# 2025-comprehensive-design/AudioLDM-with-LoRA

Hardware: AMD Instinct MI355X
Metric: unet_denoise_steps_per_sec (higher is better)
Workload: dtype bf16; 1 GPU; audioldm-s-full-v2 UNet + rank-4 LoRA (q,k,v,out), DDIM 200-step schedule, batch 4 x 10 s clips (latent 250x16), CFG 2.5 (UNet batch 8), bf16; per_gpu_batch=4, parallelism=prompt-sharded x1, hip_graph=True, graph_chains=1

## Files before the change

### audioldm_with_lora_amd/csrc/attention.hip

```cpp
#include "common.h"
#include <cstdlib>
#include <type_traits>

#ifndef ATTN_ML
#define ATTN_ML 0
#endif
#ifndef ATTN_FENCE
#define ATTN_FENCE 0
#endif

namespace {

constexpr int KV = 64;
constexpr int VS = 136;
constexpr int VS8 = 72;


typedef float f32x2 __attribute__((ext_vector_type(2)));
constexpr float RESCALE_THR = 5.0f;

__device__ __forceinline__ float max3f(float a, float b, float c) {
  float d;
  asm("v_max3_f32 %0, %1, %2, %3" : "=v"(d) : "v"(a), "v"(b), "v"(c));
  return d;
}

template <int DP, bool FP8 = false>
struct AttnCfg {
  static constexpr int DK = DP / 16;
  static constexpr bool VL = DP % 32 == 0;
  static constexpr int DT = VL ? DP / 32 : DP / 32 + 1;
  static constexpr int ONES_T = VL ? 0 : DP / 32;
  static constexpr int ONES_I = 4 * ((DP % 32) >> 3);
  static_assert(DP % 16 == 0, "row DP must land on hh = 0, register 4 * (row / 8)");
  static constexpr int KS = FP8 ? DP + 8 : DP * 2 + (((DP / 8) % 2 == 0) ? 16 : 0);
  static constexpr int VSB = FP8 ? VS8 : VS;
  static constexpr int KBYTES = KV * KS;
  static constexpr int VBYTES = DT * 32 * VSB;
  static constexpr int TILE = KBYTES + VBYTES;
};

template <int DP, int NW, int SP, bool PRESCALED, bool FP8 = false, bool LSE = false>
__global__ __launch_bounds__(64 * NW) void attention_kernel(const bf16* __restrict__ q, int ldq,
                                                            const bf16* __restrict__ k, int ldk,
                                                            const bf16* __restrict__ vt, int vt_ld, long long vt_bs,
                                                            int N, int D, float c ,
                                                            bf16* __restrict__ out, int out_ld, float* __restrict__ lse,
                                                            const int* __restrict__ kv_len) {
  aldm_touch_kernargs<96>();
#ifndef ALDM_NO_KA_PREFETCH
  aldm_prefetch_next_kernargs<96>(threadIdx.x);
#endif
  using Cfg = AttnCfg<DP, FP8>;
  constexpr int T = 64 * NW;
  constexpr int DK = Cfg::DK, DT = Cfg::DT, KS = Cfg::KS, VS = Cfg::VSB;
#ifndef ATTN_FP8_PBIAS
#define ATTN_FP8_PBIAS 8.f
#endif
  constexpr float PBIAS = FP8 ? ATTN_FP8_PBIAS : 0.f;
  using frag_t = std::conditional_t<FP8, long, bf16x8>;
  constexpr int KCH = KV * (DP / 8);
  constexpr int VCH = DP * (KV / 8);
  constexpr int KPT = (KCH + T - 1) / T, VPT = (VCH + T - 1) / T;
  constexpr int QW = NW / SP;
  static_assert(NW % SP == 0, "waves must divide into key groups");

  extern __shared__ __attribute__((aligned(16))) char smem[];
  char* Ks = smem;
  char* Vs = smem + 2 * SP * Cfg::KBYTES;

  const int tid = threadIdx.x, lane = tid & 63, wave = tid >> 6;
  const int r = lane & 31, hh = lane >> 5;
  int qblk = blockIdx.x, head = blockIdx.y, b = blockIdx.z;
  {
    const int nq = gridDim.x, H = gridDim.y, npairs = H * gridDim.z;
    if ((npairs & 7) == 0) {
      const int L = blockIdx.x + nq * (blockIdx.y + H * blockIdx.z);
      const int xcd = L & 7, slot = L >> 3;
      const int pl = slot / nq;
      qblk = slot - pl * nq;
      const int pair = pl * 8 + xcd;
      b = pair / H;
      head = pair - b * H;
    }
  }
  const int grp = wave / QW;
  const int q0 = (qblk * QW + (wave - grp * QW)) * 32;
  const bf16* qb = q + (long long)b * N * ldq + head * D;
  const bf16* kb = k + (long long)b * N * ldk + head * D;
  const bf16* vb = vt + (long long)b * vt_bs + (long long)head * D * vt_ld;
  const bf16x8 zero8 = {0, 0, 0, 0, 0, 0, 0, 0};
  const int Nk = kv_len ? max(1, min(kv_len[b], N)) : N;
  if (kv_len && qblk * QW * 32 >= Nk) {
    for (int i = tid; i < QW * 32 * (D / 4); i += T) {
      const int row = qblk * QW * 32 + i / (D / 4), c4 = i % (D / 4);
      if (row < N) *reinterpret_cast<uint2*>(out + ((long long)b * N + row) * out_ld + head * D + c4 * 4) = make_uint2(0u, 0u);
    }
    return;
  }

  {
    const int npad = DT * 32 - D;
    for (int i = tid; i < 2 * SP * npad * (VS / 8); i += T) {
      const int buf = i / (npad * (VS / 8)), rem = i - buf * npad * (VS / 8);
      const unsigned fill = (!Cfg::VL && D + rem / (VS / 8) == DP) ? (FP8 ? 0x38383838u : 0x3F803F80u) : 0u;
      reinterpret_cast<uint2*>(Vs + buf * Cfg::VBYTES + D * VS)[rem] = make_uint2(fill, fill);
    }
  }

  frag_t qf[DK];
#pragma unroll
  for (int ks = 0; ks < DK; ++ks) {
    const int col = 16 * ks + 8 * hh;
    const bf16x8 qv = (q0 + r < N && col < D) ? *reinterpret_cast<const bf16x8*>(qb + (long long)(q0 + r) * ldq + col) : zero8;
    if constexpr (FP8) { const uint2 f = bf16x8_to_fp8(qv); qf[ks] = pack2(f.x, f.y); }
    else qf[ks] = qv;
  }

  bf16x8 kreg[2][SP][KPT], vreg[2][SP][VPT];
  constexpr unsigned OOB = 0x80000000u;
  unsigned k_off[KPT], v_off[VPT];
#pragma unroll
  for (int i = 0; i < KPT; ++i) {
    const int cidx = tid + i * T;
    const int row = cidx / (DP / 8), ch = cidx - row * (DP / 8);
    k_off[i] = (cidx < KCH && ch * 8 < D) ? (unsigned)row * (unsigned)(ldk * 2) + ch * 16 : OOB;
  }
#pragma unroll
  for (int i = 0; i < VPT; ++i) {
    const int cidx = tid + i * T;
    const int row = cidx >> 3, ch = cidx & 7;
    v_off[i] = (cidx < VCH && row < D) ? (unsigned)row * (unsigned)(vt_ld * 2) + ch * 16 : OOB;
  }
  auto prefetch_k = [&](int kvbase, auto setc) {
   constexpr int SET = decltype(setc)::value;
#pragma unroll
   for (int j = 0; j < SP; ++j) {
    const int kv0 = kvbase + j * KV;
    const int bytes = max(0, ((Nk - kv0 - 1) * ldk + D) * 2);
    const __amdgpu_buffer_rsrc_t rs = __builtin_amdgcn_make_buffer_rsrc(const_cast<bf16*>(kb + (long long)kv0 * ldk), 0, kv0 < Nk ? bytes : 0, 0x00020000);
#pragma unroll
    for (int i = 0; i < KPT; ++i) kreg[SET][j][i] = __builtin_bit_cast(bf16x8, __builtin_amdgcn_raw_buffer_load_b128(rs, k_off[i], 0, 0));
   }
  };
  auto prefetch_v = [&](int kvbase, auto setc) {
   constexpr int SET = decltype(setc)::value;
#pragma unroll
   for (int j = 0; j < SP; ++j) {
    const int kv0 = kvbase + j * KV;
    const int bytes = max(0, (D * vt_ld - kv0) * 2);
    const __amdgpu_buffer_rsrc_t rs = __builtin_amdgcn_make_buffer_rsrc(const_cast<bf16*>(vb + kv0), 0, kv0 < Nk ? bytes : 0, 0x00020000);
#pragma unroll
    for (int i = 0; i < VPT; ++i) vreg[SET][j][i] = __builtin_bit_cast(bf16x8, __builtin_amdgcn_raw_buffer_load_b128(rs, v_off[i], 0, 0));
   }
  };
  auto prefetch = [&](int kvbase, auto setc) { prefetch_k(kvbase, setc); prefetch_v(kvbase, setc); };
  auto stage_k = [&](int buf, auto setc) {
   constexpr int SET = decltype(setc)::value;
#pragma unroll
   for (int j = 0; j < SP; ++j) {
#pragma unroll
    for (int i = 0; i < KPT; ++i) {
      const int cidx = tid + i * T;
      const int row = cidx / (DP / 8), ch = cidx - row * (DP / 8);
      if (cidx < KCH) {
        if constexpr (FP8) *reinterpret_cast<uint2*>(Ks + (buf * SP + j) * Cfg::KBYTES + row * KS + ch * 8) = bf16x8_to_fp8(kreg[SET][j][i]);
        else *reinterpret_cast<bf16x8*>(Ks + (buf * SP + j) * Cfg::KBYTES + row * KS + ch * 16) = kreg[SET][j][i];
      }
    }
   }
  };
  auto stage_v = [&](int buf, auto setc, int kvbase) {
   constexpr int SET = decltype(setc)::value;
#pragma unroll
   for (int j = 0; j < SP; ++j) {
    const int kv0 = kvbase + j * KV;
#pragma unroll
    for (int i = 0; i < VPT; ++i) {
      const int cidx = tid + i * T;
      const int row = cidx >> 3, ch = cidx & 7;
      if (cidx < VCH) {
        bf16x8 v = vreg[SET][j][i];
        if (kv0 + KV > Nk) {
#pragma unroll
          for (int e = 0; e < 8; ++e) if (kv0 + ch * 8 + e >= Nk) v[e] = (bf16)0.f;
        }
        if constexpr (FP8) {
          *reinterpret_cast<uint2*>(Vs + (buf * SP + j) * Cfg::VBYTES + row * VS + ch * 8) = bf16x8_to_fp8(v);
        } else {
          uint2* dst = reinterpret_cast<uint2*>(Vs + (buf * SP + j) * Cfg::VBYTES + row * VS + ch * 16);
          const uint4 u = __builtin_bit_cast(uint4, v);
          dst[0] = make_uint2(u.x, u.y);
          dst[1] = make_uint2(u.z, u.w);
        }
      }
    }
   }
  };
  auto stage = [&](int buf, auto setc, int kvbase) { stage_k(buf, setc); stage_v(buf, setc, kvbase); };

  f32x16 o[DT];
#pragma unroll
  for (int t = 0; t < DT; ++t)
#pragma unroll
    for (int i = 0; i < 16; ++i) o[t][i] = 0.f;
  float m_run = 0.f;
  constexpr bool ML = Cfg::VL && ATTN_ML;
  constexpr bool LSUM = LSE && !Cfg::VL;
  static_assert(!(LSE && (FP8 || PRESCALED)), "the lse form is the plain bf16 kernel");
  float l_run = 0.f;
  f32x2 l_pk = {0.f, 0.f};
  f32x16 lacc;
#pragma unroll
  for (int i = 0; i < 16; ++i) lacc[i] = 0.f;
  const bf16x8 ones8 = {(bf16)1.f, (bf16)1.f, (bf16)1.f, (bf16)1.f, (bf16)1.f, (bf16)1.f, (bf16)1.f, (bf16)1.f};
  f32x16 minit;
#pragma unroll
  for (int i = 0; i < 16; ++i) minit[i] = 0.f;

  const int ntiles = (Nk + KV - 1) / KV;
  const int niter = (ntiles + SP - 1) / SP;
  using Set0 = std::integral_constant<int, 0>;
  using Set1 = std::integral_constant<int, 1>;

  auto scores = [&](int it, f32x16 (&s)[2]) {
    const int buf = (it & 1) * SP + grp;
#pragma unroll
    for (int sub = 0; sub < 2; ++sub) {
#pragma unroll
      for (int ks = 0; ks < DK; ++ks) {
        if constexpr (FP8) {
          const uint2 kf = *reinterpret_cast<const uint2*>(Ks + buf * Cfg::KBYTES + (sub * 32 + r) * KS + 16 * ks + 8 * hh);
// ... 70 lines not shown
        const uint2 hi = *reinterpret_cast<const uint2*>(vrow + 16);
        return __builtin_bit_cast(bf16x8, make_uint4(lo.x, lo.y, hi.x, hi.y));
      }
    };
    frag_t vf[2][DT];
#pragma unroll
    for (int t = 0; t < DT; ++t) vf[0][t] = vfrag(t, 0);
#pragma unroll
    for (int s2 = 0; s2 < 4; ++s2) {
      const int sub = s2 >> 1, i0 = (s2 & 1) * 8;
      if (s2 + 1 < 4) {
#pragma unroll
        for (int t = 0; t < DT; ++t) vf[(s2 + 1) & 1][t] = vfrag(t, s2 + 1);
      }
      int pw8[2] = {0, 0};
#pragma unroll
      for (int i = 0; i < 8; i += 2) {
        const float e0 = PRESCALED ? s[sub][i0 + i] : fmaf(s[sub][i0 + i], c, PBIAS - m_run);
        const float e1 = PRESCALED ? s[sub][i0 + i + 1] : fmaf(s[sub][i0 + i + 1], c, PBIAS - m_run);
#ifdef ATTN_DIAG_NOEXP
        const float p0 = e0, p1 = e1;
#else
        const float p0 = __builtin_amdgcn_exp2f(e0), p1 = __builtin_amdgcn_exp2f(e1);
#endif
#ifdef ATTN_FP8_CLAMP
        const float p0c = fminf(p0, 448.f), p1c = fminf(p1, 448.f);
#define P0 p0c
#define P1 p1c
#else
#define P0 p0
#define P1 p1
#endif
        if constexpr ((Cfg::VL && !ML) || LSUM) l_pk += f32x2{p0, p1};
        if constexpr (FP8) {
          pw8[i >> 2] = (i & 2) ? __builtin_amdgcn_cvt_pk_fp8_f32(P0, P1, pw8[i >> 2], true) : __builtin_amdgcn_cvt_pk_fp8_f32(P0, P1, pw8[i >> 2], false);
        } else {
          pf[s2][i] = (bf16)p0;
          pf[s2][i + 1] = (bf16)p1;
        }
      }
      if constexpr (FP8) pf[s2] = pack2((unsigned)pw8[0], (unsigned)pw8[1]);
      if (ATTN_FENCE) __builtin_amdgcn_sched_barrier(0);
#pragma unroll
      for (int t = 0; t < DT; ++t) {
        if constexpr (FP8) o[t] = __builtin_amdgcn_mfma_f32_32x32x16_fp8_fp8(vf[s2 & 1][t], pf[s2], o[t], 0, 0, 0);
        else o[t] = __builtin_amdgcn_mfma_f32_32x32x16_bf16(vf[s2 & 1][t], pf[s2], o[t], 0, 0, 0);
      }
      if constexpr (ML && !FP8) lacc = __builtin_amdgcn_mfma_f32_32x32x16_bf16(ones8, pf[s2], lacc, 0, 0, 0);
      if (ATTN_FENCE) __builtin_amdgcn_sched_barrier(0);
    }
  };
  auto mine = [&](int it) { return SP == 1 || (it * SP + grp) * KV < Nk; };

  prefetch(0, Set0{});
  prefetch(SP * KV, Set1{});
  stage(0, Set0{}, 0);
  __builtin_amdgcn_s_waitcnt(0x0F70);
  __syncthreads();
  auto iteration = [&](int it, auto curc) {
    constexpr int CUR = decltype(curc)::value;
    f32x16 s[2];
    const bool me = mine(it);
#if ATTN_FENCE
    if (me) scores(it, s);
    __builtin_amdgcn_sched_barrier(0);
    if (it + 1 < niter) stage((it & 1) ^ 1, std::integral_constant<int, CUR ^ 1>{}, (it + 1) * SP * KV);
    prefetch((it + 2) * SP * KV, curc);
    __builtin_amdgcn_sched_barrier(0);
    if (me) softmax_pv(it, s);
#else
#ifndef ATTN_DIAG_NOLOAD
    prefetch((it + 2) * SP * KV, curc);
#endif
    if (me) {
      scores(it, s);
      softmax_pv(it, s);
    }
#ifndef ATTN_DIAG_NOLOAD
    if (it + 1 < niter) stage((it & 1) ^ 1, std::integral_constant<int, CUR ^ 1>{}, (it + 1) * SP * KV);
#endif
#endif
    __syncthreads();
  };
  for (int it = 0; it < niter; it += 2) {
    iteration(it, Set0{});
    if (it + 1 < niter) iteration(it + 1, Set1{});
  }
  if constexpr ((Cfg::VL && !ML) || LSUM) l_run = l_pk[0] + l_pk[1];

  if constexpr (SP > 1) {
    constexpr int WVALS = DT * 16 + 2;
    float* xch = reinterpret_cast<float*>(smem);
    const bool idle = grp * KV >= Nk;
    if (grp > 0) {
      float* mine = xch + ((grp - 1) * QW + (wave - grp * QW)) * WVALS * 64;
      mine[lane] = idle ? -INFINITY : m_run;
#pragma unroll
      for (int t = 0; t < DT; ++t)
#pragma unroll
        for (int i = 0; i < 16; ++i) mine[(1 + t * 16 + i) * 64 + lane] = o[t][i];
      mine[(1 + DT * 16) * 64 + lane] = ML ? lacc[0] : l_run;
    }
    __syncthreads();
    if (grp > 0) return;
#pragma unroll
    for (int g = 1; g < SP; ++g) {
      const float* peer = xch + ((g - 1) * QW + wave) * WVALS * 64;
      const float m1 = peer[lane];
      const float m_new = fmaxf(m_run, m1);
      const float a0 = __builtin_amdgcn_exp2f(m_run - m_new), a1 = __builtin_amdgcn_exp2f(m1 - m_new);
      m_run = m_new;
#pragma unroll
      for (int t = 0; t < DT; ++t)
#pragma unroll
        for (int i = 0; i < 16; ++i) o[t][i] = o[t][i] * a0 + peer[(1 + t * 16 + i) * 64 + lane] * a1;
      lacc[0] = lacc[0] * a0 + peer[(1 + DT * 16) * 64 + lane] * a1;
      l_run = l_run * a0 + peer[(1 + DT * 16) * 64 + lane] * a1;
    }
  }

  const float l_half = (Cfg::VL && !ML) ? l_run : o[Cfg::ONES_T][Cfg::ONES_I];
  const float l_tot = ML ? lacc[0] : l_half + __shfl_xor(l_half, 32, 64);
  const float inv = 1.0f / l_tot;
  const float l_lse = LSUM ? l_run + __shfl_xor(l_run, 32, 64) : l_tot;
  if (lse && hh == 0 && q0 + r < N)
    lse[((long long)b * gridDim.y + head) * N + q0 + r] = m_run + __log2f(l_lse);
  if (q0 + r < N) {
    bf16* orow = out + ((long long)b * N + q0 + r) * out_ld + head * D;
#pragma unroll
    for (int t = 0; t < (DP + 31) / 32; ++t)
#pragma unroll
      for (int g = 0; g < 4; ++g) {
        const int d0 = t * 32 + 8 * g + 4 * hh;
        if (d0 < D) {
          bf16x4 v = {(bf16)(o[t][4 * g] * inv), (bf16)(o[t][4 * g + 1] * inv), (bf16)(o[t][4 * g + 2] * inv), (bf16)(o[t][4 * g + 3] * inv)};
          *reinterpret_cast<bf16x4*>(orow + d0) = v;
        }
      }
  }
}

template <int DP, int NW, int SP, bool PS, bool FP8 = false, bool LSE = false>
int launch_attn(const void* q, int ldq, const void* k, int ldk, const void* vt, int vt_ld, long long vt_bs, int B, int N,
                int H, int D, float scale, void* out, int out_ld, float* lse, const int* kv_len, hipStream_t st) {
  using Cfg = AttnCfg<DP, FP8>;
  auto kern = attention_kernel<DP, NW, SP, PS, FP8, LSE>;
  constexpr int MERGE = SP == 1 ? 0 : (SP - 1) * (NW / SP) * (Cfg::DT * 16 + 2) * 256;
  constexpr int LDS = 2 * SP * Cfg::TILE > MERGE ? 2 * SP * Cfg::TILE : MERGE;
  static unsigned long long attr_done = 0;
  if (LDS > 48 * 1024)
    if (int rc = aldm_set_max_lds(reinterpret_cast<const void*>(kern), LDS, &attr_done, "attention")) return rc;
  dim3 grid(cdiv(N, 32 * (NW / SP)), H, B);
  hipLaunchKernelGGL(kern, grid, dim3(64 * NW), LDS, st, (const bf16*)q, ldq, (const bf16*)k, ldk, (const bf16*)vt,
                     vt_ld, vt_bs, N, D, scale * 1.44269504088896340736f, (bf16*)out, out_ld, lse, kv_len);
  return aldm_launch_status("attention");
}

template <int DP, bool PS, bool FP8 = false>
int launch_attn_d(const void* q, int ldq, const void* k, int ldk, const void* vt, int vt_ld, long long vt_bs, int B, int N,
                  int H, int D, float scale, void* out, int out_ld, float* lse, const int* kv_len, hipStream_t st) {
#define ALDM_ATTN_ARGS q, ldq, k, ldk, vt, vt_ld, vt_bs, B, N, H, D, scale, out, out_ld, lse, kv_len, st
  if constexpr (FP8) {
    if (N >= 768) {
      if ((long long)cdiv(N, 256) * H * B >= 256) return launch_attn<DP, 8, 1, PS, true>(ALDM_ATTN_ARGS);
      return launch_attn<DP, 8, 2, PS, true>(ALDM_ATTN_ARGS);
    }
    if (N >= 192) return launch_attn<DP, 4, 2, PS, true>(ALDM_ATTN_ARGS);
    if (N >= 64) return launch_attn<DP, 4, 1, PS, true>(ALDM_ATTN_ARGS);
    return launch_attn<DP, 1, 1, PS, true>(ALDM_ATTN_ARGS);
  }
#define ALDM_ATTN_GO(NWV, SPV)                                                              \
  do {                                                                                      \
    if constexpr (!PS && DP % 32 != 0) {                                                    \
      if (lse) return launch_attn<DP, NWV, SPV, PS, false, true>(ALDM_ATTN_ARGS);           \
    }                                                                                       \
    return launch_attn<DP, NWV, SPV, PS>(ALDM_ATTN_ARGS);                                   \
  } while (0)
  static const int force = getenv("ALDM_ATTN_CFG") ? atoi(getenv("ALDM_ATTN_CFG")) : 0;
  if (force == 81) ALDM_ATTN_GO(8, 1);
  if (force == 82) ALDM_ATTN_GO(8, 2);
  if (force == 41) ALDM_ATTN_GO(4, 1);
  if (force == 42) ALDM_ATTN_GO(4, 2);
  if (force == 21) ALDM_ATTN_GO(2, 1);
  if constexpr (DP == 32) {
    if (force == 162) return launch_attn<DP, 16, 2, PS>(ALDM_ATTN_ARGS);
  }
  if (N >= 768) {
    if ((long long)cdiv(N, 256) * H * B >= 256) ALDM_ATTN_GO(8, 1);
    ALDM_ATTN_GO(8, 2);
  }
  if (N >= 192) ALDM_ATTN_GO(4, 2);
  if (N >= 64) ALDM_ATTN_GO(4, 1);
  ALDM_ATTN_GO(1, 1);
#undef ALDM_ATTN_GO
#undef ALDM_ATTN_ARGS
}

__global__ __launch_bounds__(256) void softmax_rows_kernel(const float* __restrict__ s, int rows, int cols, int ld_in,
                                                           float c, bf16* __restrict__ p, int ld_out) {
  __shared__ float red[8];
  const int row = blockIdx.x, tid = threadIdx.x;
  const float* sr = s + (long long)row * ld_in;
  float mx = -INFINITY;
  for (int i = tid; i < cols; i += 256) mx = fmaxf(mx, sr[i]);
  mx = wave_max(mx);
  if ((tid & 63) == 0) red[tid >> 6] = mx;
  __syncthreads();
  mx = fmaxf(fmaxf(red[0], red[1]), fmaxf(red[2], red[3]));
  float sum = 0.f;
  for (int i = tid; i < cols; i += 256) sum += __builtin_amdgcn_exp2f((sr[i] - mx) * c);
  sum = wave_sum(sum);
  if ((tid & 63) == 0) red[4 + (tid >> 6)] = sum;
  __syncthreads();
  const float inv = 1.0f / (red[4] + red[5] + red[6] + red[7]);
  bf16* pr = p + (long long)row * ld_out;
  for (int i = tid; i < ld_out; i += 256) pr[i] = i < cols ? (bf16)(__builtin_amdgcn_exp2f((sr[i] - mx) * c) * inv) : (bf16)0.f;
}

}

template <bool PS, bool FP8 = false>
static int attention_impl(const void* q, int ldq, const void* k, int ldk, const void* vt, int vt_ld,
                          long long vt_batch_stride, int B, int N, int H, int d, float scale, void* out, int out_ld,
                          float* lse, const int* kv_len, void* stream) {
  ALDM_CHECK_ARG(q && k && vt && out, "attention: null pointer");
  ALDM_CHECK_ARG(B > 0 && N > 0 && H > 0 && d > 0, "attention: bad dims");
  ALDM_CHECK_ARG(d % 8 == 0 && ldq % 8 == 0 && ldk % 8 == 0 && vt_ld % 8 == 0 && out_ld % 4 == 0, "attention: d/ld must be multiples of 8");
  ALDM_CHECK_ARG(vt_ld >= ((N + 7) / 8) * 8, "attention: vt_ld %d too small for N %d", vt_ld, N);
  hipStream_t st = (hipStream_t)stream;
#define ALDM_ATTN(DPV) return launch_attn_d<DPV, PS, FP8>(q, ldq, k, ldk, vt, vt_ld, vt_batch_stride, B, N, H, d, scale, out, out_ld, lse, kv_len, st)
  if (d <= 16) ALDM_ATTN(16);
  if (d <= 32) ALDM_ATTN(32);
  if (d <= 48) ALDM_ATTN(48);
  if (d <= 64) ALDM_ATTN(64);
  if (d <= 80) ALDM_ATTN(80);
#undef ALDM_ATTN
  aldm_set_error("attention: head dim %d > 80 is handled by the GEMM path", d);
  return ALDM_E_UNSUPPORTED;
}

extern "C" int aldm_attention(const void* q, int ldq, const void* k, int ldk, const void* vt, int vt_ld,
                              long long vt_batch_stride, int B, int N, int H, int d, float scale, void* out, int out_ld,
                              void* stream) {
  return attention_impl<false>(q, ldq, k, ldk, vt, vt_ld, vt_batch_stride, B, N, H, d, scale, out, out_ld, nullptr, nullptr, stream);
}

extern "C" int aldm_attention_prescaled(const void* q, int ldq, const void* k, int ldk, const void* vt, int vt_ld,
// ... 34 lines not shown
```

### audioldm_with_lora_amd/csrc/attn_block64.hip

```cpp
#include "igemm_core.h"

namespace {

using aldm_igemm_detail::lds_ptr_t;
using aldm_igemm_detail::wait_vmcnt;

struct Blk64Args {
  const bf16* x;
  const float* ln_parts;
  const bf16* w;
  const float* bias;
  const float* ln_s;
  const bf16* lora_a;
  const bf16* lora_b;
  const float* ln_sa;
  const float* ln_ca;
  bf16* out;
  int np, Kpad, Rp, N, H;
  float eps;
  unsigned long long* diag;
  const float* gate;
};

#ifdef ALDM_B64_DIAG
#define B64_STAMP(i) if (p.diag && blockIdx.x == 0 && blockIdx.y == 0 && tid == 0) { unsigned long long t_; asm volatile("s_memtime %0\n\ts_waitcnt lgkmcnt(0)" : "=s"(t_) :: "memory"); p.diag[i] = t_; }
#else
#define B64_STAMP(i)
#endif

typedef unsigned int u32x4 __attribute__((ext_vector_type(4)));

template <int C, int D, int RT , bool F8 = false, bool GATED = false>
__global__ __launch_bounds__(256) void attn_block64_kernel(const Blk64Args p) {
#if defined(__HIP_DEVICE_COMPILE__)
  aldm_touch_kernargs<sizeof(Blk64Args)>();
#ifndef ALDM_NO_KA_PREFETCH
  aldm_prefetch_next_kernargs<sizeof(Blk64Args)>(threadIdx.x);
#endif
  constexpr int NTOK = 64, CPR = C / 8;
  constexpr int KSTEPS = C / 32;
  constexpr int DTL = D / 16;
  constexpr int NTILES = RT + 3 * DTL;
  constexpr int DKS = (D + 31) / 32;
  constexpr int KSTR = D * 2 + 16;
  constexpr int VSTR = NTOK * 2 + 8;
  constexpr int WTILE = 16 * C * 2, WSTAGE = WTILE + 1024;
  constexpr int P = 5;
  constexpr int NS = 3;
  static_assert(CPR % 16 == 0 && D % 16 == 0 && WTILE / 1024 == 20, "C = 640; D % 16 == 0");
  extern __shared__ __attribute__((aligned(16))) char smem[];
  char* const Wr = smem;
  char* const Ks = Wr + NS * WSTAGE;
  char* const Vt = Ks + NTOK * KSTR;
  float* const sn_l = reinterpret_cast<float*>(Vt + D * VSTR);
  float* const cn_l = sn_l + 3 * D;

  const int tid = threadIdx.x, lane = tid & 63;
  const int wave = __builtin_amdgcn_readfirstlane(tid >> 6);
  const int n = lane & 15, g = lane >> 4;
  const int head = blockIdx.x, b = blockIdx.y;
  const int N = p.N;
  const long long row0 = (long long)b * N;
  const int tok = 16 * wave + n;
  const bool live = tok < N;
  B64_STAMP(0)

  const __amdgpu_buffer_rsrc_t rs_x = aldm_igemm_detail::make_rsrc(p.x + row0 * C, (unsigned)(N * C * 2));
  const __amdgpu_buffer_rsrc_t rs_w = aldm_igemm_detail::make_rsrc(p.w, (unsigned)(3u * C * (unsigned)p.Kpad * 2u));
  const __amdgpu_buffer_rsrc_t rs_a = aldm_igemm_detail::make_rsrc(RT ? (const void*)p.lora_a : (const void*)p.w, (unsigned)((RT ? p.Rp : 16) * p.Kpad * 2));
  const __amdgpu_buffer_rsrc_t rs_b = aldm_igemm_detail::make_rsrc(RT ? (const void*)p.lora_b : (const void*)p.w, (unsigned)(RT ? 3u * C * (unsigned)p.Rp * 2u : 64u));

  float ln_a = 0.f, ln_q = 0.f;
  if (live) {
    const float* pp = p.ln_parts + (row0 + tok) * (p.np * 2);
    float2 v[16];
#pragma unroll
    for (int j = 0; j < 16; ++j) v[j] = j < p.np ? *reinterpret_cast<const float2*>(pp + 2 * j) : make_float2(0.f, 0.f);
#pragma unroll
    for (int j = 0; j < 16; ++j) { ln_a += v[j].x; ln_q += v[j].y; }
  }
  float sn_v = 0.f, cn_v = 0.f;
  if (tid < 3 * D) {
    const int sec = tid / D, r = tid - sec * D;
    sn_v = p.ln_s[sec * C + head * D + r];
    cn_v = p.bias[sec * C + head * D + r];
  }
  f32x4 sa[RT ? RT : 1], ca[RT ? RT : 1];
#pragma unroll
  for (int t = 0; t < RT; ++t) {
    sa[t] = *reinterpret_cast<const f32x4*>(p.ln_sa + 16 * t + 4 * g);
    ca[t] = *reinterpret_cast<const f32x4*>(p.ln_ca + 16 * t + 4 * g);
  }
  f32x4 gt[(GATED && RT) ? RT : 1];
  if constexpr (GATED) {
#pragma unroll
    for (int t = 0; t < RT; ++t) gt[t] = *reinterpret_cast<const f32x4*>(p.gate + (long long)b * p.Rp + 16 * t + 4 * g);
  }
  __builtin_amdgcn_sched_barrier(0);
  bf16x8 xf[KSTEPS];
#pragma unroll
  for (int ks = 0; ks < KSTEPS; ++ks)
    xf[ks] = __builtin_bit_cast(bf16x8, __builtin_amdgcn_raw_buffer_load_b128(rs_x, tok * (C * 2) + (32 * ks + 8 * g) * 2, 0, 0));
  __builtin_amdgcn_sched_barrier(0);

  auto wrow0 = [&](int t) {
    const int j = t - RT, sec = j / DTL, jj = j - sec * DTL;
    return sec * C + head * D + 16 * jj;
  };
  int w_src[5], w_dst[5];
#pragma unroll
  for (int i = 0; i < 5; ++i) {
    const int c = (wave + 4 * i) * 64 + lane, row = c / CPR, ph = c - row * CPR;
    w_src[i] = row * (p.Kpad * 2) + ph * 16;
    w_dst[i] = row * (C * 2) + ((ph ^ (row & 15)) * 16);
  }
  const int b_src = (lane >> 2) * (p.Rp * 2) + (lane & 3) * 16;
  u32x4 wreg[P][5], breg[P];
  auto gload = [&](int t) {
    const int slot = t % P;
    const bool la = t < RT;
    const int r0 = la ? 16 * t : wrow0(t);
    const int base = r0 * (p.Kpad * 2);
#pragma unroll
    for (int i = 0; i < 5; ++i) wreg[slot][i] = __builtin_amdgcn_raw_buffer_load_b128(la ? rs_a : rs_w, base + w_src[i], 0, 0);
    if (RT > 0 && !la && wave == (t & 3)) breg[slot] = __builtin_amdgcn_raw_buffer_load_b128(rs_b, r0 * (p.Rp * 2) + b_src, 0, 0);
  };
  auto lstore = [&](int t) {
    const int slot = t % P;
    char* const dst = Wr + (t % NS) * WSTAGE;
#pragma unroll
    for (int i = 0; i < 5; ++i) *reinterpret_cast<u32x4*>(dst + w_dst[i]) = wreg[slot][i];
    if (RT > 0 && t >= RT && wave == (t & 3)) *reinterpret_cast<u32x4*>(dst + WTILE + lane * 16) = breg[slot];
  };
  const int w_rd = n * (C * 2);
  bf16x8 wf[2][KSTEPS];
  auto lread = [&](int t, int ks) {
    wf[t & 1][ks] = *reinterpret_cast<const bf16x8*>(Wr + (t % NS) * WSTAGE + w_rd + (((4 * ks + g) ^ n) * 16));
  };
#pragma unroll
  for (int t = 0; t < P; ++t) gload(t);
  __builtin_amdgcn_sched_barrier(0);

  float mean = 0.f, rstd = 0.f;
  if (live) {
    mean = ln_a * (1.f / C);
    rstd = rsqrtf(fmaxf(ln_q * (1.f / C) - mean * mean, 0.f) + p.eps);
  }
  if (tid < 3 * D) { sn_l[tid] = sn_v; cn_l[tid] = cn_v; }
  B64_STAMP(1)
  lstore(0);
  if (P < NTILES) gload(P);
  lstore(1);
  if (P + 1 < NTILES) gload(P + 1);
  __builtin_amdgcn_s_waitcnt(0xC07F);
  __builtin_amdgcn_s_barrier();
  B64_STAMP(2)
#pragma unroll
  for (int ks = 0; ks < KSTEPS; ++ks) lread(0, ks);
  B64_STAMP(3)

  bf16x8 tf = {0, 0, 0, 0, 0, 0, 0, 0};
  bf16x8 qf[DKS];
#pragma unroll
  for (int ks = 0; ks < DKS; ++ks) qf[ks] = bf16x8{0, 0, 0, 0, 0, 0, 0, 0};
  const float irs = rstd != 0.f ? 1.f / rstd : 0.f;

#pragma unroll
  for (int t = 0; t < NTILES; ++t) {
    if (t + 2 < NTILES) {
      lstore(t + 2);
      if (t + 2 + P < NTILES) gload(t + 2 + P);
    }
    f32x4 acc = {0.f, 0.f, 0.f, 0.f}, acc2 = {0.f, 0.f, 0.f, 0.f};
#pragma unroll
    for (int ks = 0; ks < KSTEPS; ks += 2) {
      if (t + 1 < NTILES) { lread(t + 1, ks); lread(t + 1, ks + 1); }
      acc = __builtin_amdgcn_mfma_f32_16x16x32_bf16(wf[t & 1][ks], xf[ks], acc, 0, 0, 0);
      acc2 = __builtin_amdgcn_mfma_f32_16x16x32_bf16(wf[t & 1][ks + 1], xf[ks + 1], acc2, 0, 0, 0);
    }
    acc += acc2;
    const char* Wb = Wr + (t % NS) * WSTAGE;
    if (t < RT) {
#pragma unroll
      for (int j = 0; j < 4; ++j) {
        float tv = acc[j] - mean * sa[t < RT ? t : 0][j] + ca[t < RT ? t : 0][j] * irs;
        if constexpr (GATED) tv *= gt[t < RT ? t : 0][j];
        tf[4 * t + j] = (bf16)tv;
      }
    } else {
      if (RT > 0) {
        const char* brow = Wb + WTILE + n * 64 + g * 8;
        const bf16x4 lo = *reinterpret_cast<const bf16x4*>(brow);
        const bf16x4 hi = (RT > 1) ? *reinterpret_cast<const bf16x4*>(brow + 32) : bf16x4{0, 0, 0, 0};
        acc = __builtin_amdgcn_mfma_f32_16x16x32_bf16(__builtin_shufflevector(lo, hi, 0, 1, 2, 3, 4, 5, 6, 7), tf, acc, 0, 0, 0);
      }
      const int j0 = t - RT, sec = j0 / DTL, jj = j0 - sec * DTL;
      const f32x4 sn = *reinterpret_cast<const f32x4*>(sn_l + sec * D + 16 * jj + 4 * g), cn = *reinterpret_cast<const f32x4*>(cn_l + sec * D + 16 * jj + 4 * g);
      bf16x4 y;
#pragma unroll
      for (int j = 0; j < 4; ++j) y[j] = live ? (bf16)(rstd * (acc[j] - mean * sn[j]) + cn[j]) : (bf16)0.f;
      const int dcol = 16 * jj + 4 * g;
      if (sec == 0) {
#pragma unroll
        for (int j = 0; j < 4; ++j) qf[jj >> 1][(jj & 1) * 4 + j] = y[j];
      } else if (sec == 1) {
        *reinterpret_cast<bf16x4*>(Ks + tok * KSTR + dcol * 2) = y;
      } else {
#pragma unroll
        for (int j = 0; j < 4; ++j) *reinterpret_cast<bf16*>(Vt + (dcol + j) * VSTR + tok * 2) = y[j];
      }
    }
    __builtin_amdgcn_s_waitcnt(0xC07F);
    __builtin_amdgcn_s_barrier();
    B64_STAMP(4 + t)
  }

  f32x4 s[4];
#pragma unroll
  for (int kt = 0; kt < 4; ++kt) {
    s[kt] = f32x4{0.f, 0.f, 0.f, 0.f};
#pragma unroll
    for (int ks = 0; ks < DKS; ++ks) {
      const char* krow = Ks + (16 * kt + n) * KSTR + (32 * ks + 4 * g) * 2;
      const bf16x4 lo = *reinterpret_cast<const bf16x4*>(krow);
// ... 17 lines not shown
      mx = fmaxf(mx, s[kt][j]);
    }
  mx = fmaxf(mx, __shfl_xor(mx, 16, 64));
  mx = fmaxf(mx, __shfl_xor(mx, 32, 64));
  float l = 0.f;
  bf16x8 pf[2];
  int p8[4] = {0, 0, 0, 0};
#pragma unroll
  for (int kt = 0; kt < 4; ++kt) {
    if constexpr (F8) {
      const float e0 = __builtin_amdgcn_exp2f(s[kt][0] - mx + 8.f), e1 = __builtin_amdgcn_exp2f(s[kt][1] - mx + 8.f);
      const float e2 = __builtin_amdgcn_exp2f(s[kt][2] - mx + 8.f), e3 = __builtin_amdgcn_exp2f(s[kt][3] - mx + 8.f);
      p8[kt] = __builtin_amdgcn_cvt_pk_fp8_f32(e0, e1, p8[kt], false);
      p8[kt] = __builtin_amdgcn_cvt_pk_fp8_f32(e2, e3, p8[kt], true);
      l += (__builtin_amdgcn_cvt_f32_fp8(p8[kt], 0) + __builtin_amdgcn_cvt_f32_fp8(p8[kt], 1)) +
           (__builtin_amdgcn_cvt_f32_fp8(p8[kt], 2) + __builtin_amdgcn_cvt_f32_fp8(p8[kt], 3));
    } else {
#pragma unroll
      for (int j = 0; j < 4; ++j) {
        const bf16 pb = (bf16)__builtin_amdgcn_exp2f(s[kt][j] - mx);
        l += (float)pb;
        pf[kt >> 1][(kt & 1) * 4 + j] = pb;
      }
    }
  }
  l += __shfl_xor(l, 16, 64);
  l += __shfl_xor(l, 32, 64);
  const float inv = 1.0f / l;
  B64_STAMP(22)
  bf16* orow = p.out + (row0 + tok) * C + head * D;
#pragma unroll
  for (int t = 0; t < DTL; ++t) {
    f32x4 o = {0.f, 0.f, 0.f, 0.f};
#pragma unroll
    for (int kk = 0; kk < 2; ++kk) {
      const char* vrow = Vt + (16 * t + n) * VSTR + (32 * kk + 4 * g) * 2;
      const bf16x4 lo = *reinterpret_cast<const bf16x4*>(vrow);
      const bf16x4 hi = *reinterpret_cast<const bf16x4*>(vrow + 32);
      const bf16x8 vf = __builtin_shufflevector(lo, hi, 0, 1, 2, 3, 4, 5, 6, 7);
      if constexpr (F8) {
        const uint2 v8 = bf16x8_to_fp8(vf);
        o = __builtin_amdgcn_mfma_f32_16x16x32_fp8_fp8(pack2(v8.x, v8.y), pack2((unsigned)p8[2 * kk], (unsigned)p8[2 * kk + 1]), o, 0, 0, 0);
      } else {
        o = __builtin_amdgcn_mfma_f32_16x16x32_bf16(vf, pf[kk], o, 0, 0, 0);
      }
    }
    const bf16x4 ov = {(bf16)(o[0] * inv), (bf16)(o[1] * inv), (bf16)(o[2] * inv), (bf16)(o[3] * inv)};
    if (live) *reinterpret_cast<bf16x4*>(orow + 16 * t + 4 * g) = ov;
  }
  B64_STAMP(23)
#endif
}

template <int C, int D, int RT, bool F8 = false, bool GATED = false>
int launch_blk64(const Blk64Args& a, int B, hipStream_t st) {
  constexpr int LDS = 3 * (16 * C * 2 + 1024) + 64 * (D * 2 + 16) + D * (64 * 2 + 8) + 2 * 3 * D * 4;
  static_assert(LDS <= 160 * 1024, "LDS budget");
  auto kern = attn_block64_kernel<C, D, RT, F8, GATED>;
  static unsigned long long attr_done = 0;
  if (int rc = aldm_set_max_lds(reinterpret_cast<const void*>(kern), LDS, &attr_done, "attn_block64")) return rc;
  hipLaunchKernelGGL(kern, dim3(a.H, B), dim3(256), LDS, st, a);
  return aldm_launch_status("attn_block64");
}

unsigned long long* g_b64_diag = nullptr;


}

extern "C" void aldm_attn_block64_set_diag(void* buf) { g_b64_diag = (unsigned long long*)buf; }

static int attn_block64_entry(bool f8, const void* x, const float* ln_parts, int ln_nparts, const void* w, int Kpad, const float* bias,
                                 const float* ln_s, const void* lora_a, const void* lora_b, int Rp, int ranks_used,
                                 const float* ln_sa, const float* ln_ca, float ln_eps, int B, int N, int H, int d, void* out,
                                 const float* lora_gate, void* stream) {
  ALDM_CHECK_ARG(x && ln_parts && w && bias && ln_s && out, "attn_block64: null pointer");
  ALDM_CHECK_ARG(!lora_gate || Rp, "attn_block64: lora_gate without an adapter");
  ALDM_CHECK_ARG(B > 0 && N > 0 && N <= 64 && ln_nparts > 0 && ln_nparts <= 16, "attn_block64: 1 <= N <= 64 tokens per sample, 1 <= ln_nparts <= 16");
  ALDM_CHECK_ARG(Rp == 0 || (Rp % 16 == 0 && ranks_used > 0 && ranks_used <= 32 && ranks_used <= Rp && lora_a && lora_b && ln_sa && ln_ca),
                 "attn_block64: LoRA needs Rp %% 16 == 0, 1 <= ranks_used <= min(32, Rp) and lora_a / lora_b / ln_sa / ln_ca");
  ALDM_CHECK_ARG(H == 8 && d == 80 && Kpad == 640, "attn_block64: built for C = 640 = 8 heads x 80 (the UNet's 64-token level); got H %d d %d Kpad %d", H, d, Kpad);
  Blk64Args a{(const bf16*)x, ln_parts, (const bf16*)w, bias, ln_s, (const bf16*)lora_a, (const bf16*)lora_b, ln_sa, ln_ca, (bf16*)out,
              ln_nparts, Kpad, Rp, N, H, ln_eps, g_b64_diag, lora_gate};
  hipStream_t st = (hipStream_t)stream;
  if (lora_gate) {
    if (f8) return ranks_used <= 16 ? launch_blk64<640, 80, 1, true, true>(a, B, st) : launch_blk64<640, 80, 2, true, true>(a, B, st);
    return ranks_used <= 16 ? launch_blk64<640, 80, 1, false, true>(a, B, st) : launch_blk64<640, 80, 2, false, true>(a, B, st);
  }
  if (f8) {
    if (Rp == 0) return launch_blk64<640, 80, 0, true>(a, B, st);
    if (ranks_used <= 16) return launch_blk64<640, 80, 1, true>(a, B, st);
    return launch_blk64<640, 80, 2, true>(a, B, st);
  }
  if (Rp == 0) return launch_blk64<640, 80, 0>(a, B, st);
  if (ranks_used <= 16) return launch_blk64<640, 80, 1>(a, B, st);
  return launch_blk64<640, 80, 2>(a, B, st);
}

extern "C" int aldm_attn_block64(const void* x, const float* ln_parts, int ln_nparts, const void* w, int Kpad, const float* bias,
                                 const float* ln_s, const void* lora_a, const void* lora_b, int Rp, int ranks_used,
                                 const float* ln_sa, const float* ln_ca, float ln_eps, int B, int N, int H, int d, void* out,
                                 void* stream) {
  return attn_block64_entry(false, x, ln_parts, ln_nparts, w, Kpad, bias, ln_s, lora_a, lora_b, Rp, ranks_used, ln_sa, ln_ca, ln_eps, B, N, H, d, out, nullptr, stream);
}
extern "C" int aldm_attn_block64_fp8(const void* x, const float* ln_parts, int ln_nparts, const void* w, int Kpad, const float* bias,
                                     const float* ln_s, const void* lora_a, const void* lora_b, int Rp, int ranks_used,
                                     const float* ln_sa, const float* ln_ca, float ln_eps, int B, int N, int H, int d, void* out,
                                     void* stream) {
  return attn_block64_entry(true, x, ln_parts, ln_nparts, w, Kpad, bias, ln_s, lora_a, lora_b, Rp, ranks_used, ln_sa, ln_ca, ln_eps, B, N, H, d, out, nullptr, stream);
}
extern "C" int aldm_attn_block64_gated(const void* x, const float* ln_parts, int ln_nparts, const void* w, int Kpad, const float* bias,
                                       const float* ln_s, const void* lora_a, const void* lora_b, int Rp, int ranks_used,
                                       const float* ln_sa, const float* ln_ca, float ln_eps, int B, int N, int H, int d, void* out,
                                       void* stream, const float* lora_gate) {
  ALDM_CHECK_ARG(lora_gate, "attn_block64_gated: null lora_gate");
// ... 10 lines not shown
```

Measured before the change: 351.3 denoise_steps/s.

## Add dedicated loader waves to attention and attn_block64 kernels

Both attention kernels gain warp-specialized variants. Extra waves do only the global-to-LDS prefetch and staging of K/V tiles, or of weight tiles in attn_block64. The compute waves then only run MFMA and softmax work, with barriers handing off each tile. The aim is to take load-issue latency and register pressure off the compute waves. The cost is larger workgroups, which may lower occupancy and add barrier overhead. Both paths are on by default (attention only for N>=192) and can be turned off through environment variables.

```diff
diff --git a/audioldm_with_lora_amd/csrc/attention.hip b/audioldm_with_lora_amd/csrc/attention.hip
--- a/audioldm_with_lora_amd/csrc/attention.hip
+++ b/audioldm_with_lora_amd/csrc/attention.hip
@@ -40,8 +40,8 @@
   static constexpr int TILE = KBYTES + VBYTES;
 };
 
-template <int DP, int NW, int SP, bool PRESCALED, bool FP8 = false, bool LSE = false>
-__global__ __launch_bounds__(64 * NW) void attention_kernel(const bf16* __restrict__ q, int ldq,
+template <int DP, int NW, int SP, bool PRESCALED, bool FP8 = false, bool LSE = false, int NL = 0>
+__global__ __launch_bounds__(64 * (NW + NL)) void attention_kernel(const bf16* __restrict__ q, int ldq,
                                                             const bf16* __restrict__ k, int ldk,
                                                             const bf16* __restrict__ vt, int vt_ld, long long vt_bs,
                                                             int N, int D, float c ,
@@ -52,7 +52,8 @@
   aldm_prefetch_next_kernargs<96>(threadIdx.x);
 #endif
   using Cfg = AttnCfg<DP, FP8>;
-  constexpr int T = 64 * NW;
+  constexpr int T = NL ? 64 * NL : 64 * NW;
+  constexpr int TALL = 64 * (NW + NL);
   constexpr int DK = Cfg::DK, DT = Cfg::DT, KS = Cfg::KS, VS = Cfg::VSB;
 #ifndef ATTN_FP8_PBIAS
 #define ATTN_FP8_PBIAS 8.f
@@ -69,7 +70,11 @@
   char* Ks = smem;
   char* Vs = smem + 2 * SP * Cfg::KBYTES;
 
-  const int tid = threadIdx.x, lane = tid & 63, wave = tid >> 6;
+  const int tid = threadIdx.x, lane = tid & 63;
+  int wave = tid >> 6;
+  if constexpr (NL > 0) wave = __builtin_amdgcn_readfirstlane(wave);
+  const bool loader = NL > 0 && wave >= NW;
+  const int stid = NL ? tid - 64 * NW : tid;
   const int r = lane & 31, hh = lane >> 5;
   int qblk = blockIdx.x, head = blockIdx.y, b = blockIdx.z;
   {
@@ -92,16 +97,16 @@
   const bf16x8 zero8 = {0, 0, 0, 0, 0, 0, 0, 0};
   const int Nk = kv_len ? max(1, min(kv_len[b], N)) : N;
   if (kv_len && qblk * QW * 32 >= Nk) {
-    for (int i = tid; i < QW * 32 * (D / 4); i += T) {
+    for (int i = tid; i < QW * 32 * (D / 4); i += TALL) {
       const int row = qblk * QW * 32 + i / (D / 4), c4 = i % (D / 4);
       if (row < N) *reinterpret_cast<uint2*>(out + ((long long)b * N + row) * out_ld + head * D + c4 * 4) = make_uint2(0u, 0u);
     }
     return;
   }
 
-  {
+  if (NL == 0 || loader) {
     const int npad = DT * 32 - D;
-    for (int i = tid; i < 2 * SP * npad * (VS / 8); i += T) {
+    for (int i = stid; i < 2 * SP * npad * (VS / 8); i += T) {
       const int buf = i / (npad * (VS / 8)), rem = i - buf * npad * (VS / 8);
       const unsigned fill = (!Cfg::VL && D + rem / (VS / 8) == DP) ? (FP8 ? 0x38383838u : 0x3F803F80u) : 0u;
       reinterpret_cast<uint2*>(Vs + buf * Cfg::VBYTES + D * VS)[rem] = make_uint2(fill, fill);
@@ -112,7 +117,7 @@
 #pragma unroll
   for (int ks = 0; ks < DK; ++ks) {
     const int col = 16 * ks + 8 * hh;
-    const bf16x8 qv = (q0 + r < N && col < D) ? *reinterpret_cast<const bf16x8*>(qb + (long long)(q0 + r) * ldq + col) : zero8;
+    const bf16x8 qv = (!loader && q0 + r < N && col < D) ? *reinterpret_cast<const bf16x8*>(qb + (long long)(q0 + r) * ldq + col) : zero8;
     if constexpr (FP8) { const uint2 f = bf16x8_to_fp8(qv); qf[ks] = pack2(f.x, f.y); }
     else qf[ks] = qv;
   }
@@ -122,13 +127,13 @@
   unsigned k_off[KPT], v_off[VPT];
 #pragma unroll
   for (int i = 0; i < KPT; ++i) {
-    const int cidx = tid + i * T;
+    const int cidx = stid + i * T;
     const int row = cidx / (DP / 8), ch = cidx - row * (DP / 8);
     k_off[i] = (cidx < KCH && ch * 8 < D) ? (unsigned)row * (unsigned)(ldk * 2) + ch * 16 : OOB;
   }
 #pragma unroll
   for (int i = 0; i < VPT; ++i) {
-    const int cidx = tid + i * T;
+    const int cidx = stid + i * T;
     const int row = cidx >> 3, ch = cidx & 7;
     v_off[i] = (cidx < VCH && row < D) ? (unsigned)row * (unsigned)(vt_ld * 2) + ch * 16 : OOB;
   }
@@ -161,7 +166,7 @@
    for (int j = 0; j < SP; ++j) {
 #pragma unroll
     for (int i = 0; i < KPT; ++i) {
-      const int cidx = tid + i * T;
+      const int cidx = stid + i * T;
       const int row = cidx / (DP / 8), ch = cidx - row * (DP / 8);
       if (cidx < KCH) {
         if constexpr (FP8) *reinterpret_cast<uint2*>(Ks + (buf * SP + j) * Cfg::KBYTES + row * KS + ch * 8) = bf16x8_to_fp8(kreg[SET][j][i]);
@@ -177,7 +182,7 @@
     const int kv0 = kvbase + j * KV;
 #pragma unroll
     for (int i = 0; i < VPT; ++i) {
-      const int cidx = tid + i * T;
+      const int cidx = stid + i * T;
       const int row = cidx >> 3, ch = cidx & 7;
       if (cidx < VCH) {
         bf16x8 v = vreg[SET][j][i];
@@ -354,39 +359,74 @@
   };
   auto mine = [&](int it) { return SP == 1 || (it * SP + grp) * KV < Nk; };
 
-  prefetch(0, Set0{});
-  prefetch(SP * KV, Set1{});
-  stage(0, Set0{}, 0);
-  __builtin_amdgcn_s_waitcnt(0x0F70);
-  __syncthreads();
-  auto iteration = [&](int it, auto curc) {
-    constexpr int CUR = decltype(curc)::value;
-    f32x16 s[2];
-    const bool me = mine(it);
+  if constexpr (NL > 0) {
+    if (loader) {
+      prefetch(0, Set0{});
+      prefetch(SP * KV, Set1{});
+      stage(0, Set0{}, 0);
+      __syncthreads();
+      auto feed = [&](int it, auto curc) __attribute__((always_inline)) {
+        constexpr int CUR = decltype(curc)::value;
+        prefetch((it + 2) * SP * KV, curc);
+        if (it + 1 < niter) stage((it & 1) ^ 1, std::integral_constant<int, CUR ^ 1>{}, (it + 1) * SP * KV);
+        __syncthreads();
+      };
+      for (int it = 0; it < niter; it += 2) {
+        feed(it, Set0{});
+        if (it + 1 < niter) feed(it + 1, Set1{});
+      }
+      if constexpr (SP > 1) __syncthreads();
+      return;
+    }
+    __builtin_amdgcn_s_waitcnt(0x0F70);
+    __syncthreads();
+    auto tile = [&](int it) __attribute__((always_inline)) {
+      f32x16 s[2];
+      if (mine(it)) {
+        scores(it, s);
+        softmax_pv(it, s);
+      }
+      __syncthreads();
+    };
+    for (int it = 0; it < niter; it += 2) {
+      tile(it);
+      if (it + 1 < niter) tile(it + 1);
+    }
+  } else {
+    prefetch(0, Set0{});
+    prefetch(SP * KV, Set1{});
+    stage(0, Set0{}, 0);
+    __builtin_amdgcn_s_waitcnt(0x0F70);
+    __syncthreads();
+    auto iteration = [&](int it, auto curc) {
+      constexpr int CUR = decltype(curc)::value;
+      f32x16 s[2];
+      const bool me = mine(it);
 #if ATTN_FENCE
-    if (me) scores(it, s);
-    __builtin_amdgcn_sched_barrier(0);
-    if (it + 1 < niter) stage((it & 1) ^ 1, std::integral_constant<int, CUR ^ 1>{}, (it + 1) * SP * KV);
-    prefetch((it + 2) * SP * KV, curc);
-    __builtin_amdgcn_sched_barrier(0);
-    if (me) softmax_pv(it, s);
+      if (me) scores(it, s);
+      __builtin_amdgcn_sched_barrier(0);
+      if (it + 1 < niter) stage((it & 1) ^ 1, std::integral_constant<int, CUR ^ 1>{}, (it + 1) * SP * KV);
+      prefetch((it + 2) * SP * KV, curc);
+      __builtin_amdgcn_sched_barrier(0);
+      if (me) softmax_pv(it, s);
 #else
 #ifndef ATTN_DIAG_NOLOAD
-    prefetch((it + 2) * SP * KV, curc);
-#endif
-    if (me) {
-      scores(it, s);
-      softmax_pv(it, s);
-    }
+      prefetch((it + 2) * SP * KV, curc);
+#endif
+      if (me) {
+        scores(it, s);
+        softmax_pv(it, s);
+      }
 #ifndef ATTN_DIAG_NOLOAD
-    if (it + 1 < niter) stage((it & 1) ^ 1, std::integral_constant<int, CUR ^ 1>{}, (it + 1) * SP * KV);
-#endif
-#endif
-    __syncthreads();
-  };
-  for (int it = 0; it < niter; it += 2) {
-    iteration(it, Set0{});
-    if (it + 1 < niter) iteration(it + 1, Set1{});
+      if (it + 1 < niter) stage((it & 1) ^ 1, std::integral_constant<int, CUR ^ 1>{}, (it + 1) * SP * KV);
+#endif
+#endif
+      __syncthreads();
+    };
+    for (int it = 0; it < niter; it += 2) {
+      iteration(it, Set0{});
+      if (it + 1 < niter) iteration(it + 1, Set1{});
+    }
   }
   if constexpr ((Cfg::VL && !ML) || LSUM) l_run = l_pk[0] + l_pk[1];
 
@@ -442,33 +482,48 @@
   }
 }
 
-template <int DP, int NW, int SP, bool PS, bool FP8 = false, bool LSE = false>
+template <int DP, int NW, int SP, bool PS, bool FP8 = false, bool LSE = false, int NL = 0>
 int launch_attn(const void* q, int ldq, const void* k, int ldk, const void* vt, int vt_ld, long long vt_bs, int B, int N,
                 int H, int D, float scale, void* out, int out_ld, float* lse, const int* kv_len, hipStream_t st) {
   using Cfg = AttnCfg<DP, FP8>;
-  auto kern = attention_kernel<DP, NW, SP, PS, FP8, LSE>;
+  auto kern = attention_kernel<DP, NW, SP, PS, FP8, LSE, NL>;
   constexpr int MERGE = SP == 1 ? 0 : (SP - 1) * (NW / SP) * (Cfg::DT * 16 + 2) * 256;
   constexpr int LDS = 2 * SP * Cfg::TILE > MERGE ? 2 * SP * Cfg::TILE : MERGE;
   static unsigned long long attr_done = 0;
   if (LDS > 48 * 1024)
     if (int rc = aldm_set_max_lds(reinterpret_cast<const void*>(kern), LDS, &attr_done, "attention")) return rc;
   dim3 grid(cdiv(N, 32 * (NW / SP)), H, B);
-  hipLaunchKernelGGL(kern, grid, dim3(64 * NW), LDS, st, (const bf16*)q, ldq, (const bf16*)k, ldk, (const bf16*)vt,
+  hipLaunchKernelGGL(kern, grid, dim3(64 * (NW + NL)), LDS, st, (const bf16*)q, ldq, (const bf16*)k, ldk, (const bf16*)vt,
                      vt_ld, vt_bs, N, D, scale * 1.44269504088896340736f, (bf16*)out, out_ld, lse, kv_len);
   return aldm_launch_status("attention");
+}
+
+constexpr int ATTN_NL = 4;
+inline int attn_loaders(int N) {
+  const char* e = getenv("ALDM_ATTN_LOADERS");
+  const int v = e ? atoi(e) : -1;
+  if (v == 0) return 0;
+  if (v == ATTN_NL) return N >= 64 ? ATTN_NL : 0;
+  return N >= 192 ? ATTN_NL : 0;
 }
 
 template <int DP, bool PS, bool FP8 = false>
 int launch_attn_d(const void* q, int ldq, const void* k, int ldk, const void* vt, int vt_ld, long long vt_bs, int B, int N,
                   int H, int D, float scale, void* out, int out_ld, float* lse, const int* kv_len, hipStream_t st) {
 #define ALDM_ATTN_ARGS q, ldq, k, ldk, vt, vt_ld, vt_bs, B, N, H, D, scale, out, out_ld, lse, kv_len, st
+  const int nl = attn_loaders(N);
+#define ALDM_ATTN_NL(NWV, SPV, F8V, LSEV)                                                   \
+  do {                                                                                      \
+    if (nl) return launch_attn<DP, NWV, SPV, PS, F8V, LSEV, ATTN_NL>(ALDM_ATTN_ARGS);       \
+    return launch_attn<DP, NWV, SPV, PS, F8V, LSEV>(ALDM_ATTN_ARGS);                        \
+  } while (0)
   if constexpr (FP8) {
     if (N >= 768) {
-      if ((long long)cdiv(N, 256) * H * B >= 256) return launch_attn<DP, 8, 1, PS, true>(ALDM_ATTN_ARGS);
-      return launch_attn<DP, 8, 2, PS, true>(ALDM_ATTN_ARGS);
-    }
-    if (N >= 192) return launch_attn<DP, 4, 2, PS, true>(ALDM_ATTN_ARGS);
-    if (N >= 64) return launch_attn<DP, 4, 1, PS, true>(ALDM_ATTN_ARGS);
+      if ((long long)cdiv(N, 256) * H * B >= 256) ALDM_ATTN_NL(8, 1, true, false);
+      ALDM_ATTN_NL(8, 2, true, false);
+    }
+    if (N >= 192) ALDM_ATTN_NL(4, 2, true, false);
+    if (N >= 64) ALDM_ATTN_NL(4, 1, true, false);
     return launch_attn<DP, 1, 1, PS, true>(ALDM_ATTN_ARGS);
   }
 #define ALDM_ATTN_GO(NWV, SPV)                                                              \
@@ -477,6 +532,13 @@
       if (lse) return launch_attn<DP, NWV, SPV, PS, false, true>(ALDM_ATTN_ARGS);           \
     }                                                                                       \
     return launch_attn<DP, NWV, SPV, PS>(ALDM_ATTN_ARGS);                                   \
+  } while (0)
+#define ALDM_ATTN_GOL(NWV, SPV)    \
+  do {                                                                                      \
+    if constexpr (!PS && DP % 32 != 0) {                                                    \
+      if (lse) ALDM_ATTN_NL(NWV, SPV, false, true);                                         \
+    }                                                                                       \
+    ALDM_ATTN_NL(NWV, SPV, false, false);                                                   \
   } while (0)
   static const int force = getenv("ALDM_ATTN_CFG") ? atoi(getenv("ALDM_ATTN_CFG")) : 0;
   if (force == 81) ALDM_ATTN_GO(8, 1);
@@ -488,13 +550,15 @@
     if (force == 162) return launch_attn<DP, 16, 2, PS>(ALDM_ATTN_ARGS);
   }
   if (N >= 768) {
-    if ((long long)cdiv(N, 256) * H * B >= 256) ALDM_ATTN_GO(8, 1);
-    ALDM_ATTN_GO(8, 2);
-  }
-  if (N >= 192) ALDM_ATTN_GO(4, 2);
-  if (N >= 64) ALDM_ATTN_GO(4, 1);
+    if ((long long)cdiv(N, 256) * H * B >= 256) ALDM_ATTN_GOL(8, 1);
+    ALDM_ATTN_GOL(8, 2);
+  }
+  if (N >= 192) ALDM_ATTN_GOL(4, 2);
+  if (N >= 64) ALDM_ATTN_GOL(4, 1);
   ALDM_ATTN_GO(1, 1);
 #undef ALDM_ATTN_GO
+#undef ALDM_ATTN_GOL
+#undef ALDM_ATTN_NL
 #undef ALDM_ATTN_ARGS
 }
 
diff --git a/audioldm_with_lora_amd/csrc/attn_block64.hip b/audioldm_with_lora_amd/csrc/attn_block64.hip
--- a/audioldm_with_lora_amd/csrc/attn_block64.hip
+++ b/audioldm_with_lora_amd/csrc/attn_block64.hip
@@ -1,4 +1,5 @@
 #include "igemm_core.h"
+#include <cstdlib>
 
 namespace {
 
@@ -29,9 +30,10 @@
 #endif
 
 typedef unsigned int u32x4 __attribute__((ext_vector_type(4)));
-
-template <int C, int D, int RT , bool F8 = false, bool GATED = false>
-__global__ __launch_bounds__(256) void attn_block64_kernel(const Blk64Args p) {
+constexpr bool B64_LOADERS_DEFAULT = true;
+
+template <int C, int D, int RT , bool F8 = false, bool GATED = false, bool LW = false>
+__global__ __launch_bounds__(LW ? 512 : 256) void attn_block64_kernel(const Blk64Args p) {
 #if defined(__HIP_DEVICE_COMPILE__)
   aldm_touch_kernargs<sizeof(Blk64Args)>();
 #ifndef ALDM_NO_KA_PREFETCH
@@ -61,8 +63,10 @@
   const int head = blockIdx.x, b = blockIdx.y;
   const int N = p.N;
   const long long row0 = (long long)b * N;
+  const bool loader = LW && wave >= 4;
+  const int lw = LW ? wave - 4 : wave;
   const int tok = 16 * wave + n;
-  const bool live = tok < N;
+  const bool live = !loader && tok < N;
   B64_STAMP(0)
 
   const __amdgpu_buffer_rsrc_t rs_x = aldm_igemm_detail::make_rsrc(p.x + row0 * C, (unsigned)(N * C * 2));
@@ -87,19 +91,19 @@
   }
   f32x4 sa[RT ? RT : 1], ca[RT ? RT : 1];
 #pragma unroll
-  for (int t = 0; t < RT; ++t) {
+  for (int t = 0; t < RT && !loader; ++t) {
     sa[t] = *reinterpret_cast<const f32x4*>(p.ln_sa + 16 * t + 4 * g);
     ca[t] = *reinterpret_cast<const f32x4*>(p.ln_ca + 16 * t + 4 * g);
   }
   f32x4 gt[(GATED && RT) ? RT : 1];
   if constexpr (GATED) {
 #pragma unroll
-    for (int t = 0; t < RT; ++t) gt[t] = *reinterpret_cast<const f32x4*>(p.gate + (long long)b * p.Rp + 16 * t + 4 * g);
+    for (int t = 0; t < RT && !loader; ++t) gt[t] = *reinterpret_cast<const f32x4*>(p.gate + (long long)b * p.Rp + 16 * t + 4 * g);
   }
   __builtin_amdgcn_sched_barrier(0);
   bf16x8 xf[KSTEPS];
 #pragma unroll
-  for (int ks = 0; ks < KSTEPS; ++ks)
+  for (int ks = 0; ks < KSTEPS && !loader; ++ks)
     xf[ks] = __builtin_bit_cast(bf16x8, __builtin_amdgcn_raw_buffer_load_b128(rs_x, tok * (C * 2) + (32 * ks + 8 * g) * 2, 0, 0));
   __builtin_amdgcn_sched_barrier(0);
 
@@ -110,7 +114,7 @@
   int w_src[5], w_dst[5];
 #pragma unroll
   for (int i = 0; i < 5; ++i) {
-    const int c = (wave + 4 * i) * 64 + lane, row = c / CPR, ph = c - row * CPR;
+    const int c = (lw + 4 * i) * 64 + lane, row = c / CPR, ph = c - row * CPR;
     w_src[i] = row * (p.Kpad * 2) + ph * 16;
     w_dst[i] = row * (C * 2) + ((ph ^ (row & 15)) * 16);
   }
@@ -123,22 +127,45 @@
     const int base = r0 * (p.Kpad * 2);
 #pragma unroll
     for (int i = 0; i < 5; ++i) wreg[slot][i] = __builtin_amdgcn_raw_buffer_load_b128(la ? rs_a : rs_w, base + w_src[i], 0, 0);
-    if (RT > 0 && !la && wave == (t & 3)) breg[slot] = __builtin_amdgcn_raw_buffer_load_b128(rs_b, r0 * (p.Rp * 2) + b_src, 0, 0);
+    if (RT > 0 && !la && lw == (t & 3)) breg[slot] = __builtin_amdgcn_raw_buffer_load_b128(rs_b, r0 * (p.Rp * 2) + b_src, 0, 0);
   };
   auto lstore = [&](int t) {
     const int slot = t % P;
     char* const dst = Wr + (t % NS) * WSTAGE;
 #pragma unroll
     for (int i = 0; i < 5; ++i) *reinterpret_cast<u32x4*>(dst + w_dst[i]) = wreg[slot][i];
-    if (RT > 0 && t >= RT && wave == (t & 3)) *reinterpret_cast<u32x4*>(dst + WTILE + lane * 16) = breg[slot];
+    if (RT > 0 && t >= RT && lw == (t & 3)) *reinterpret_cast<u32x4*>(dst + WTILE + lane * 16) = breg[slot];
   };
   const int w_rd = n * (C * 2);
   bf16x8 wf[2][KSTEPS];
   auto lread = [&](int t, int ks) {
     wf[t & 1][ks] = *reinterpret_cast<const bf16x8*>(Wr + (t % NS) * WSTAGE + w_rd + (((4 * ks + g) ^ n) * 16));
   };
-#pragma unroll
-  for (int t = 0; t < P; ++t) gload(t);
+  if constexpr (LW) {
+    if (loader) {
+#pragma unroll
+      for (int t = 0; t < P; ++t) gload(t);
+      lstore(0);
+      if (P < NTILES) gload(P);
+      lstore(1);
+      if (P + 1 < NTILES) gload(P + 1);
+      __builtin_amdgcn_s_waitcnt(0xC07F);
+      __builtin_amdgcn_s_barrier();
+#pragma unroll
+      for (int t = 0; t < NTILES; ++t) {
+        if (t + 2 < NTILES) {
+          lstore(t + 2);
+          if (t + 2 + P < NTILES) gload(t + 2 + P);
+        }
+        __builtin_amdgcn_s_waitcnt(0xC07F);
+        __builtin_amdgcn_s_barrier();
+      }
+      return;
+    }
+  } else {
+#pragma unroll
+    for (int t = 0; t < P; ++t) gload(t);
+  }
   __builtin_amdgcn_sched_barrier(0);
 
   float mean = 0.f, rstd = 0.f;
@@ -148,10 +175,12 @@
   }
   if (tid < 3 * D) { sn_l[tid] = sn_v; cn_l[tid] = cn_v; }
   B64_STAMP(1)
-  lstore(0);
-  if (P < NTILES) gload(P);
-  lstore(1);
-  if (P + 1 < NTILES) gload(P + 1);
+  if constexpr (!LW) {
+    lstore(0);
+    if (P < NTILES) gload(P);
+    lstore(1);
+    if (P + 1 < NTILES) gload(P + 1);
+  }
   __builtin_amdgcn_s_waitcnt(0xC07F);
   __builtin_amdgcn_s_barrier();
   B64_STAMP(2)
@@ -167,9 +196,11 @@
 
 #pragma unroll
   for (int t = 0; t < NTILES; ++t) {
-    if (t + 2 < NTILES) {
-      lstore(t + 2);
-      if (t + 2 + P < NTILES) gload(t + 2 + P);
+    if constexpr (!LW) {
+      if (t + 2 < NTILES) {
+        lstore(t + 2);
+        if (t + 2 + P < NTILES) gload(t + 2 + P);
+      }
     }
     f32x4 acc = {0.f, 0.f, 0.f, 0.f}, acc2 = {0.f, 0.f, 0.f, 0.f};
 #pragma unroll
@@ -293,15 +324,22 @@
 #endif
 }
 
+template <int C, int D, int RT, bool F8, bool GATED, bool LW>
+int launch_blk64_form(const Blk64Args& a, int B, hipStream_t st) {
+  constexpr int LDS = 3 * (16 * C * 2 + 1024) + 64 * (D * 2 + 16) + D * (64 * 2 + 8) + 2 * 3 * D * 4;
+  static_assert(LDS <= 160 * 1024, "LDS budget");
+  auto kern = attn_block64_kernel<C, D, RT, F8, GATED, LW>;
+  static unsigned long long attr_done = 0;
+  if (int rc = aldm_set_max_lds(reinterpret_cast<const void*>(kern), LDS, &attr_done, "attn_block64")) return rc;
+  hipLaunchKernelGGL(kern, dim3(a.H, B), dim3(LW ? 512 : 256), LDS, st, a);
+  return aldm_launch_status("attn_block64");
+}
+
 template <int C, int D, int RT, bool F8 = false, bool GATED = false>
 int launch_blk64(const Blk64Args& a, int B, hipStream_t st) {
-  constexpr int LDS = 3 * (16 * C * 2 + 1024) + 64 * (D * 2 + 16) + D * (64 * 2 + 8) + 2 * 3 * D * 4;
-  static_assert(LDS <= 160 * 1024, "LDS budget");
-  auto kern = attn_block64_kernel<C, D, RT, F8, GATED>;
-  static unsigned long long attr_done = 0;
-  if (int rc = aldm_set_max_lds(reinterpret_cast<const void*>(kern), LDS, &attr_done, "attn_block64")) return rc;
-  hipLaunchKernelGGL(kern, dim3(a.H, B), dim3(256), LDS, st, a);
-  return aldm_launch_status("attn_block64");
+  const char* e = getenv("ALDM_B64_LOADERS");
+  if (e && atoi(e) == 0) return launch_blk64_form<C, D, RT, F8, GATED, false>(a, B, st);
+  return launch_blk64_form<C, D, RT, F8, GATED, B64_LOADERS_DEFAULT>(a, B, st);
 }
 
 unsigned long long* g_b64_diag = nullptr;
```

New measurement: 357.3 denoise_steps/s (median of 6 runs). 1.7% higher.
